# kowallus/mbgc

Hardware: AMD Instinct MI355X
Metric: input Gbases/s (compress hot path, -m1: match-finding + stream emission) (higher is better)
Workload: dtype u8

## Files before the change

mbgc_amd/csrc/swsem_kernels.hip:

```cpp
#include "swsem_device.h"

namespace swk {


__global__ void __launch_bounds__(256) k_load_rc(const uint8_t *__restrict__ src, uint8_t *__restrict__ dst,
                                                 uint64_t n, const uint8_t *__restrict__ lut) {
    __shared__ uint8_t slut[256];
    slut[threadIdx.x] = lut[threadIdx.x];
    __syncthreads();
    const uint64_t stride = (uint64_t) gridDim.x * blockDim.x * 4;
    for (uint64_t d = ((uint64_t) blockIdx.x * blockDim.x + threadIdx.x) * 4; d < n; d += stride) {
        const uint64_t m = n - d < 4 ? n - d : 4;
#pragma unroll
        for (uint64_t k = 0; k < 4; k++)
            if (k < m) dst[d + k] = slut[src[n - 1 - d - k]];
    }
}

__global__ void k_set_byte(uint8_t *p, uint8_t v) { *p = v; }
__global__ void k_touch() {}
__global__ void __launch_bounds__(256) k_hog(unsigned long long ticks) {
    const unsigned long long t0 = __builtin_amdgcn_s_memrealtime();
    while (__builtin_amdgcn_s_memrealtime() - t0 < ticks) __builtin_amdgcn_s_sleep(8);
}
// ... 47 lines not shown
}
__global__ void k_set_bytes(uint8_t *__restrict__ ref, const BytePiece *__restrict__ b, int n, const uint32_t *__restrict__ gate) {
    if (gate && *gate == 0) return;
    for (int i = 0; i < n; i++) ref[b[i].off] = (uint8_t) b[i].val;
}
struct SumRun { uint32_t first, count, val, pad; };
__global__ void __launch_bounds__(256) k_set_tagsum(uint16_t *__restrict__ tagSum, uint32_t nEntries, const SumRun *__restrict__ runs, int n,
                                                    const uint32_t *__restrict__ gate) {
    if (gate && *gate == 0) return;
    for (int i = 0; i < n; i++) {
        const SumRun r = runs[i];
        for (uint32_t k = blockIdx.x * blockDim.x + threadIdx.x; k < r.count; k += gridDim.x * blockDim.x)
            if ((uint64_t) r.first + k < nEntries) tagSum[r.first + k] = (uint16_t) r.val;
    }
}


__device__ __forceinline__ uint32_t fp_at(const uint8_t *s, int nw) {
    uint32_t f = FP_SEED;
    for (int j = 0; j < nw; j++) f = fp_step(f, ld_u32(s + 4 * j));
    return f;
}

__global__ void __launch_bounds__(256) k_insert(const uint8_t *__restrict__ ref, ht_entry *__restrict__ ht,
                                                uint64_t S, uint64_t nMain, uint64_t T, uint64_t nTail, int k1,
                                                int k1ord, int K, uint32_t mask, uint32_t epoch, int fpBits,
                                                uint16_t *__restrict__ tags, uint32_t tag) {
    const uint64_t t = (uint64_t) blockIdx.x * blockDim.x + threadIdx.x;
    if (t >= nMain + nTail) return;
    const bool tail = t >= nMain;
    const uint64_t p = tail ? T + (t - nMain) * (uint64_t) k1 : S + t * (uint64_t) k1;
    if (tags && (p & ((1ull << k1ord) - 1)) == 0) tags[p >> k1ord] = (uint16_t) tag;
    const uint8_t *s = ref + p;
    uint32_t h = (uint32_t) K, f = FP_SEED;
    const int nw = K / 4;
    for (int j = 0; j < nw; j++) { const uint32_t w = ld_u32(s + 4 * j); h = hash_step(h, w, (uint32_t) j); f = fp_step(f, w); }
    const uint32_t off = (uint32_t) (p & ((1ull << k1ord) - 1));
    if (off && p >= off) f = fp_at(s - off, nw);
    const ht_entry key = ht_key(epoch + (tail ? 1u : 0u), (uint32_t) (p >> k1ord), f, fpBits);
    atomicMax(&ht[h & mask], key);
}

struct InsertPiece { uint64_t S, nMain, T, nTail; uint32_t epoch, tag; const uint8_t *src; uint64_t lo, hi; };
__device__ __forceinline__ bool insert_sample(const InsertPiece *__restrict__ pieces, const uint64_t *__restrict__ first, int np, int k1, uint64_t g,
                                              InsertPiece &pc, uint64_t &p, bool &tail) {
    int lo = 0, hi = np;
    while (hi - lo > 1) { const int mid = (lo + hi) / 2; if (first[mid] <= g) lo = mid; else hi = mid; }
    pc = pieces[lo];
    const uint64_t t = g - first[lo];
    tail = t >= pc.nMain;
    p = tail ? pc.T + (t - pc.nMain) * (uint64_t) k1 : pc.S + t * (uint64_t) k1;
    return true;
}
template<bool FROM_SRC>
__global__ void __launch_bounds__(256) k_insert_multi(const uint8_t *__restrict__ ref, ht_entry *__restrict__ ht,
                                                      const InsertPiece *__restrict__ pieces, const uint64_t *__restrict__ first,
                                                      int np, int k1, int k1ord, int K, uint32_t mask, int fpBits,
                                                      const uint32_t *__restrict__ gate, uint16_t *__restrict__ tags) {
    if (gate && *gate == 0) return;
    const uint64_t total = first[np];
    for (uint64_t g0 = (uint64_t) blockIdx.x * blockDim.x + threadIdx.x; g0 < total; g0 += (uint64_t) gridDim.x * blockDim.x) {
        const uint64_t g = total - 1 - g0;
        InsertPiece pc; uint64_t p; bool tail;
        insert_sample(pieces, first, np, k1, g, pc, p, tail);
        const uint8_t *s = ref + p;
        if (FROM_SRC) {
            if (!pc.src || p < pc.lo || p + (uint64_t) K > pc.hi) continue;
            s = pc.src + (p - pc.lo);
        }
        if (tags && (p & ((1ull << k1ord) - 1)) == 0) tags[p >> k1ord] = (uint16_t) pc.tag;
        uint32_t h = (uint32_t) K, f = FP_SEED;
        const int nw = K / 4;
        for (int j = 0; j < nw; j++) { const uint32_t w = ld_u32(s + 4 * j); h = hash_step(h, w, (uint32_t) j); f = fp_step(f, w); }
        const uint32_t off = (uint32_t) (p & ((1ull << k1ord) - 1));
        if (off && p >= off && (!FROM_SRC || p - off >= pc.lo)) f = fp_at(s - off, nw);
        const ht_entry key = ht_key(pc.epoch + (tail ? 1u : 0u), (uint32_t) (p >> k1ord), f, fpBits);
        const ht_entry seen = ht[h & mask];
        if (seen >= key) continue;
        atomicMax(&ht[h & mask], key);
    }
}
__global__ void k_mark_stale(const uint8_t *__restrict__ ref, ht_entry *__restrict__ ht, uint64_t p, int K, int k1ord, uint32_t mask, int fpBits,
                             uint16_t *__restrict__ tags) {
    if (tags) tags[p >> k1ord] = 0;
    uint32_t h = (uint32_t) K;
    for (int j = 0; j < K / 4; j++) h = hash_step(h, ld_u32(ref + p + 4 * j), (uint32_t) j);
    const ht_entry e = ht[h & mask];
    if ((uint32_t) (e >> fpBits) == (uint32_t) (p >> k1ord) && e != 0)
        ht[h & mask] = e & ((((ht_entry) 1) << (32 + fpBits)) - 1);
}

__global__ void __launch_bounds__(256) k_ht_low_words(const ht_entry *__restrict__ ht, uint32_t *__restrict__ out, uint64_t n, int fpBits) {
    const uint64_t i = (uint64_t) blockIdx.x * blockDim.x + threadIdx.x;
    if (i < n) out[i] = (uint32_t) (ht[i] >> fpBits);
}

struct Chain {
    int32_t scan;
    int32_t minTouched;
    int32_t minKeep;
    int32_t visited;
    uint32_t cands;
    bool emitted;
#ifdef SWSEM_DIAG_PHASES
    uint64_t tRefill, tVisit, tLcp;
    uint32_t nRefill, nLcp;
#endif
};
#ifdef SWSEM_DIAG_PHASES
__device__ unsigned long long g_diag[8];
#endif

constexpr int RING = 64;

__device__ __forceinline__ uint32_t rl32(uint32_t x, int lane) { return (uint32_t) __builtin_amdgcn_readlane((int) x, lane); }
__device__ __forceinline__ uint32_t rfl32(uint32_t x) { return (uint32_t) __builtin_amdgcn_readfirstlane((int) x); }
__device__ __forceinline__ uint64_t rfl64(uint64_t x) { return ((uint64_t) rfl32((uint32_t) (x >> 32)) << 32) | rfl32((uint32_t) x); }
constexpr int OVERLAP_MAX = 1024;
constexpr int SNAP = 4;

struct __attribute__((aligned(16))) Row {
    uint64_t posSrc, len, posDest;
    int64_t scanAfter;
};
__device__ __forceinline__ void put_row(Match *dst, const Match &m, int64_t) { *dst = m; }
__device__ __forceinline__ void put_row(Row *dst, const Match &m, int64_t scan) {
    Row r;
    r.posSrc = m.posSrc; r.len = m.len; r.posDest = m.posDest; r.scanAfter = scan;
    *dst = r;
}

template <class R>
// ... 917 lines not shown
```

mbgc_amd/csrc/swsem_runtime_emit.h:

```cpp
namespace {

int end_slot(swsem *h, int si) {
    EmitSlot &E = h->slot[si];
    if (!E.outstanding) return SWSEM_OK;
    HIPCHK(hipSetDevice(h->device));
    { int d = run_phase2b(h, E, false); if (d) return d; }
    HIPCHK(hipEventSynchronize(E.evDone));
    E.outstanding = false;
    const int n = E.emitN;
    E.eout.assign((const EmitOut *) E.pinE.p, (const EmitOut *) E.pinE.p + n);
    uint64_t tot = 0;
    E.hostStreamOff.assign((size_t) n * SWSEM_NSTREAMS, 0);
    for (int k = 0; k < n; k++)
        for (int st = 0; st < SWSEM_NSTREAMS; st++) {
            if (E.eout[k].unmatchedChars == UINT64_MAX) E.eout[k].size[st] = 0;
            E.hostStreamOff[(size_t) k * SWSEM_NSTREAMS + st] = tot;
            tot += E.eout[k].size[st];
        }
    E.packedBytes = tot;
    E.hostStreamsValid = false;
    if (h->emitHostCopy) {
        int r = E.next_host_streams(tot + 1);
        if (r) return r;
        if (tot) HIPCHK(hipMemcpyAsync(E.hostStreams().p, E.dEArena.p, tot, hipMemcpyDeviceToHost, h->s3()));
// ... 62 lines not shown
    h->roundTopFresh = false;
    HIPCHK(hipStreamWaitEvent(up, h->evRoundTop, 0));
    if ((r = upload(h, E.dEOwner.p, E.chunkOwner.data(), E.chunkOwner.size() * sizeof(uint32_t), up))) return r;
    if ((r = upload(h, E.dESpanOwner.p, E.spanOwner.data(), E.spanOwner.size() * sizeof(uint32_t), up))) return r;
    if ((r = upload(h, E.dECg.p, E.ecg.data(), n * sizeof(EmitContig), up)) || (r = upload(h, E.dEWhich.p, E.ewhich.data(), n * sizeof(int), up))) return r;
    E.eloaded.assign(refExtLoadedPos, refExtLoadedPos + nLoaded);
    if ((r = upload(h, E.dELoaded.p, E.eloaded.data(), nLoaded * sizeof(uint64_t), up))) return r;
    if (spec) {
        if ((r = h->dGate.reserve(4)) || (r = h->dPred.reserve(2 * (size_t) n + 64))) return r;
        if ((r = upload(h, h->dPred.p, spec->predExt, n, up)) || (r = upload(h, h->dPred.p + n, spec->predRC, n, up))) return r;
    }
    return flush_copies(h);
}

EmitView emit_book(swsem *h, EmitSlot &E, int si, const swsem_emit_params_t *p, int n, uint64_t nLoaded, bool regionsAhead) {
    EmitView v;
    v.ref = h->ref; v.qbuf = h->qdev; v.matches = h->dMatches.p; v.matchCount = h->dMatchCount.p;
    v.pos1 = (uint64_t) h->ld.pos1; v.refLength = h->refLength(); v.maxRefLength = h->maxRefLength;
    v.loaded = E.dELoaded.p; v.nLoaded = (uint32_t) nLoaded; v.p = *p;
    v.em = E.dEM.p; v.next0 = E.dENext0.p; v.removed = E.dERm.p; v.keepIdx = E.dEKeep.p;
    v.rawLp = regionsAhead ? E.dERawLp.p : nullptr; v.rawNext0 = regionsAhead ? E.dERawNext0.p : nullptr;
    v.meta = E.dEMeta.p; v.corr = E.dECorr.p; v.sz = E.dESz.p; v.arena = E.dEArena.p; v.out = E.dEOut.p;
    v.packBase = E.dEPack.p;
    v.pairMask = E.dEPm.p; v.litBits = E.dELit.p; v.metaBad = E.dEBad.p;
    v.longCopies = E.dELong.p; v.longCount = E.dELongCount.p;
    v.ofs = E.dEOfs.p;
    v.chunkCnt = E.dEChunk.p;
    v.chunkOwner = E.dEOwner.p; v.spanOwner = E.dESpanOwner.p;
    v.ncontigs = (uint32_t) n;
    E.v2b = v; E.grid2b = (uint32_t) E.chunkOwner.size(); E.n2b = n;
    E.donePending = true;
    h->latest = si; h->selected = -1;
    E.outstanding = true; E.refGuarded = false; E.emitN = n; E.emitPos1 = (uint64_t) h->ld.pos1; E.qdev = h->qdev; E.params = *p;
    E.emitLaps = h->ld.laps;
    uint64_t lm = UINT64_MAX; bool all = true;
    for (int k = 0; k < n; k++) { if (E.ecg[k].lock == UINT64_MAX) all = false; else lm = std::min(lm, E.ecg[k].lock); }
    E.lockMin = all ? lm : UINT64_MAX;
    E.packedBytes = 0; E.hostStreamsValid = false;
    E.deferred2b = false;
    return v;
}

int spec_plan(swsem *h, const swsem_spec_finalize_t *spec, const uint32_t *gate, bool &planned) {
    h->specMode = true;
    int r = finalize_impl(h, spec->ntargets, spec->ext_dev, spec->ext_len, spec->addSep, spec->sep, spec->lazySeparator, spec->lockPos,
                          spec->loadedAfter, gate, true);
    h->specMode = false;
    planned = r == SWSEM_OK;
    if (r == SWSEM_ESPEC) return SWSEM_OK;
    if (r) return r;
    return prepare_inserts(h, h->streamUp);
}

int emit_pass1(swsem *h, EmitSlot &E, const EmitView &v, int n) {
    const dim3 grid2(E.grid2b);
    int r;
    HIPCHK(hipEventRecord(h->evTables, h->streamUp));
    if (v.rawLp) {
        HIPCHK(hipStreamWaitEvent(h->streamAux, h->evMatched, 0));
        HIPCHK(hipStreamWaitEvent(h->streamAux, h->evTables, 0));
        k_emit_regions_raw<<<grid2, dim3(CH), 0, h->streamAux>>>(v, E.dECg.p, E.dEWhich.p);
        HIPCHK(hipEventRecord(h->evRegions, h->streamAux));
    }
    HIPCHK(hipStreamWaitEvent(h->stream, h->evTables, 0));
    hipStream_t sP = h->stream;
    h->mark(SWSEM_K_EMIT, true, sP);
    k_emit_p1_removed<<<grid2, dim3(CH), 0, sP>>>(v, E.dECg.p, E.dEWhich.p);
    k_emit_p1_scan<<<dim3(n), dim3(CH), 0, sP>>>(v, E.dECg.p, E.dEWhich.p);
    if (v.rawLp) HIPCHK(hipStreamWaitEvent(sP, h->evRegions, 0));
    k_emit_p1_compact<<<grid2, dim3(CH), 0, sP>>>(v, E.dECg.p, E.dEWhich.p);
    k_emit_p1_finish<<<dim3(n), dim3(CH), 0, sP>>>(v, E.dECg.p);
    h->mark(SWSEM_K_EMIT, false, sP);
    HIPCHK(hipGetLastError());
    if ((r = queue_counts(h, n * sizeof(EmitOut), sP))) return r;
    if ((r = download(h, h->pin.p + h->pinExtraAt, E.dEOut.p, n * sizeof(EmitOut), sP)) || (r = flush_copies(h))) return r;
    HIPCHK(hipEventRecord(h->evP1, sP));
    return SWSEM_OK;
}

int emit_pairing(swsem *h, EmitSlot &E, const EmitView &v, int n) {
    const dim3 grid2(E.grid2b), spans((uint32_t) E.spanOwner.size());
    const size_t outBytes = n * sizeof(EmitOut);
    int r = E.pinE.reserve(outBytes, std::max<size_t>(2 * outBytes, 1 << 20));
    if (r) return r;
    HIPCHK(hipStreamWaitEvent(h->streamAux, h->evP1, 0));
    h->mark(SWSEM_K_EMIT2, true, h->streamAux);
    if (!v.rawLp) k_emit_meta_regions<<<grid2, dim3(CH), 0, h->streamAux>>>(v, E.dECg.p);
    k_emit_meta_masks<<<spans, dim3(MLANES), 0, h->streamAux>>>(v, E.dECg.p);
    k_emit_meta_spec<<<spans, dim3(MLANES), 0, h->streamAux>>>(v, E.dECg.p, E.dEStates.p, h->sw.metaWarm, E.dEStat.p);
    HIPCHK(hipEventRecord(h->evMeta, h->streamAux));
    h->metaPending = true;
    k_emit_meta_check<<<grid2, dim3(WAVE), 0, h->streamAux>>>(v, E.dECg.p, E.dEStates.p, E.dEStat.p);
    k_emit_meta_stitch<<<dim3(n), dim3(WAVE), 0, h->streamAux>>>(v, E.dECg.p, E.dEStates.p, E.dEStat.p);
    h->mark(SWSEM_K_EMIT2, false, h->streamAux);
    HIPCHK(hipEventRecord(E.evMetaDone, h->streamAux));
    HIPCHK(hipGetLastError());
    return SWSEM_OK;
}

int spec_gate(swsem *h, EmitSlot &E, const swsem_spec_finalize_t *spec, uint32_t *gate, int n, bool planned, bool &queued, bool &exchanged) {
    k_spec_verify<<<1, 256, 0, h->stream>>>(E.dEOut.p, E.dECg.p, n, h->dPred.p, h->dPred.p + n, spec->factor, spec->rcFactor, gate);
    if (spec->veto || !planned) HIPCHK(hipMemsetAsync(gate, 0, sizeof(uint32_t), h->stream));
    if (spec->exchange) {
        if (spec->exchange(spec->exchange_ctx, 0, gate, (void *) h->stream)) return fail(SWSEM_EHIP, "speculative finalize: the exchange between the replicas failed");
        exchanged = true;
    }
    if (planned) {
        int r = launch_inserts(h, gate);
        if (r) return r;
        queued = true;
    }
    return SWSEM_OK;
}

bool spec_verdict(swsem *h, const EmitSlot &E, const swsem_spec_finalize_t *spec, int n, bool exchanged) {
    bool ok = !spec->veto;
    for (int k = 0; k < n && ok; k++) {
        const uint64_t un = E.eout[k].unmatchedChars, len = E.ecg[k].n;
        ok = un != UINT64_MAX && (un * (uint64_t) spec->factor > len) == (spec->predExt[k] != 0) &&
             (un * (uint64_t) spec->rcFactor > len) == (spec->predRC[k] != 0);
    }
    if (exchanged) ok = spec->exchange(spec->exchange_ctx, 1, nullptr, (void *) h->stream) == 1 && ok;
    return ok;
}

int emit_begin_impl(swsem *h, const swsem_emit_params_t *p, int n, const int *contigIdx, const uint64_t *lockPos,
                    const int *factor, const int64_t *processed, const int64_t *targetIdx,
                    const uint64_t *refExtLoadedPos, uint64_t nLoaded, const swsem_spec_finalize_t *spec, int *applied) {
    HIPCHK(hipSetDevice(h->device));
    if (applied) *applied = 0;
    if (spec && spec->ntargets <= 0) spec = nullptr;
    const int si = h->latest ^ 1;
    { int e = end_slot(h, si); if (e) return e; }
    EmitSlot &E = h->slot[si];
    if (!h->batchValid) return fail(SWSEM_EINVAL, "swsem_emit: no match results on the handle");
    if (n <= 0) return fail(SWSEM_EINVAL, "swsem_emit: empty request");
    if (p->lazyDecompressionSupport && nLoaded == 0) return fail(SWSEM_EINVAL, "swsem_emit: lazy mode needs refExtLoadedPosArr");
    if (p->gapDepthOffsetEncoding > 64 || p->gapDepthOffsetEncoding < 0)
        return fail(SWSEM_EINVAL, "gapDepthOffsetEncoding %d out of range (MAX_GAP_DEPTH / 2)", p->gapDepthOffsetEncoding);
    int r;
    uint64_t rows, arena;
    const bool regionsAhead = h->roundTopFresh && p->lazyDecompressionSupport;
    if ((r = emit_layout(h, E, n, contigIdx, lockPos, factor, processed, targetIdx, rows, arena)) ||
        (r = emit_reserve(h, E, n, rows, arena, nLoaded)) ||
        (r = emit_upload_tables(h, E, n, refExtLoadedPos, nLoaded, spec)))
        return r;
    const EmitView v = emit_book(h, E, si, p, n, nLoaded, regionsAhead);
    const LoaderState snap = h->ld;
    bool planned = false, queued = false, exchanged = false;
    uint32_t *gate = spec ? (spec->gate_dev ? spec->gate_dev : h->dGate.p) : nullptr;
    if (spec && (r = spec_plan(h, spec, gate, planned))) return r;
    const bool needCounts = h->matchCount.size() != h->contigs.size();
    if ((r = emit_pass1(h, E, v, n))) return r;
    if ((r = emit_pairing(h, E, v, n))) return r;
    if (spec) {
        if ((r = spec_gate(h, E, spec, gate, n, planned, queued, exchanged))) return r;
        if (!queued) h->ld = snap;
    }
    E.deferred2b = true; E.waitFin2b = queued;
    if (h->emitHostCopy) { int e = end_slot(h, si ^ 1); if (e) return e; }
    HIPCHK(hipEventSynchronize(h->evP1));
    if (needCounts) take_counts(h);
    E.eout.assign((const EmitOut *) (h->pin.p + h->pinExtraAt), (const EmitOut *) (h->pin.p + h->pinExtraAt) + n);
    if (queued) {
        if (spec_verdict(h, E, spec, n, exchanged)) { if (applied) *applied = 1; }
        else h->ld = snap;
    } else if (exchanged)
        (void) spec->exchange(spec->exchange_ctx, 1, nullptr, (void *) h->stream);
    return SWSEM_OK;
}

}
```

mbgc_amd/csrc/swsem_runtime_loader.h:

```cpp
namespace {

int flush_copies(swsem *h) {
    CopySegs &sg = h->segs;
    if (sg.n == 0) return SWSEM_OK;
    const uint32_t blocks = sg.first[sg.n];
    k_copy_segs<<<dim3(blocks), dim3(256), 0, h->segStream>>>(sg);
    sg.n = 0;
    HIPCHK(hipGetLastError());
    return SWSEM_OK;
}
int stage_copy(swsem *h, void *dst, const void *src, size_t bytes, hipStream_t st) {
    if (!bytes) return SWSEM_OK;
    CopySegs &sg = h->segs;
    if (sg.n && (h->segStream != st || sg.n == CopySegs::MAX)) { int r = flush_copies(h); if (r) return r; }
    if (sg.n == 0) { h->segStream = st; sg.first[0] = 0; }
    sg.dst[sg.n] = (uint8_t *) dst; sg.src[sg.n] = (const uint8_t *) src; sg.bytes[sg.n] = bytes;
    sg.first[sg.n + 1] = sg.first[sg.n] + (uint32_t) ((bytes + 4095) / 4096);
    sg.n++;
    return SWSEM_OK;
}
int download(swsem *h, void *dstPinned, const void *srcDev, size_t bytes, hipStream_t st) { return stage_copy(h, dstPinned, srcDev, bytes, st); }
int zero_dev(swsem *h, void *dst, size_t bytes, hipStream_t st) { return stage_copy(h, dst, nullptr, bytes, st); }

int upload(swsem *h, void *dst, const void *src, size_t bytes, hipStream_t st) {
// ... 232 lines not shown
    P = PreparedInserts();
    const size_t np = h->pendingPieces.size(), nc = h->pendingCopies.size(), nb = h->pendingBytes.size();
    plan_tag_summary(h, h->sumRuns);
    const size_t ns = h->sumRuns.size();
    P.np = np; P.nc = nc; P.nb = nb; P.ns = ns;
    if (!np && !nc && !nb && !ns) return SWSEM_OK;
    constexpr uint64_t CHUNK = 256 * 16;
    std::vector<InsertPiece> &edge = h->edgePieces;
    edge.clear();
    bool beside = np && nc;
    for (size_t i = 0; i < nc && beside; i++)
        for (size_t j = i + 1; j < nc && beside; j++)
            beside = h->pendingCopies[i].dst + h->pendingCopies[i].len <= h->pendingCopies[j].dst || h->pendingCopies[j].dst + h->pendingCopies[j].len <= h->pendingCopies[i].dst;
    if (beside) {
        const int64_t k1 = h->k1, K = h->K;
        for (auto &pc : h->pendingPieces) {
            if (pc.src)
                for (auto &b : h->pendingBytes)
                    if (b.off >= pc.lo && b.off < pc.hi) { if (b.off - pc.lo < pc.hi - b.off) { pc.src += b.off + 1 - pc.lo; pc.lo = b.off + 1; } else pc.hi = b.off; }
            auto runs = [&](uint64_t base, uint64_t n, uint32_t epoch) {
                if (!n) return;
                int64_t a = 0, b = -1;
                if (pc.src && (int64_t) pc.hi - K >= (int64_t) base) {
                    a = (int64_t) pc.lo > (int64_t) base ? ((int64_t) pc.lo - (int64_t) base + k1 - 1) / k1 : 0;
                    b = std::min<int64_t>((int64_t) n - 1, ((int64_t) pc.hi - K - (int64_t) base) / k1);
                }
                auto push = [&](int64_t t0, int64_t t1) {
                    if (t1 <= t0) return;
                    InsertPiece e = {};
                    e.S = base + (uint64_t) t0 * (uint64_t) k1; e.nMain = (uint64_t) (t1 - t0); e.epoch = epoch; e.tag = pc.tag;
                    edge.push_back(e);
                };
                if (b < a) push(0, (int64_t) n);
                else { push(0, a); push(b + 1, (int64_t) n); }
            };
            runs(pc.S, pc.nMain, pc.epoch);
            runs(pc.T, pc.nTail, pc.epoch + 1);
        }
    } else
        for (auto &pc : h->pendingPieces) pc.src = nullptr;
    const size_t ne = edge.size();
    const size_t wPieces = np * (sizeof(InsertPiece) / 8), wCopies = nc * (sizeof(CopyPiece) / 8), wBytes = nb * (sizeof(BytePiece) / 8), wEdge = ne * (sizeof(InsertPiece) / 8),
                 wSums = ns * (sizeof(SumRun) / 8);
    swsem::HostTab &ht = h->hostTables[h->hostTableSel ^= 1];
    const size_t words = wPieces + (np + 1) + wCopies + (nc + 1) + wBytes + wEdge + (ne + 1) + wSums;
    if (ht.pending) { HIPCHK(hipEventSynchronize(ht.ev)); ht.pending = false; }
    int r;
    if ((r = ht.buf.reserve(words * 8, std::max<size_t>(2 * words, 1 << 16) * 8))) return r;
    uint64_t *const tab = (uint64_t *) ht.buf.p;
    uint64_t *tPieces = tab, *tFirst = tPieces + wPieces, *tCopies = tFirst + np + 1, *tCFirst = tCopies + wCopies, *tBytes = tCFirst + nc + 1,
             *tEdge = tBytes + wBytes, *tEFirst = tEdge + wEdge, *tSums = tEFirst + ne + 1;
    if (np) memcpy(tPieces, h->pendingPieces.data(), np * sizeof(InsertPiece));
    tFirst[0] = 0;
    for (size_t i = 0; i < np; i++) tFirst[i + 1] = tFirst[i] + h->pendingPieces[i].nMain + h->pendingPieces[i].nTail;
    if (nc) memcpy(tCopies, h->pendingCopies.data(), nc * sizeof(CopyPiece));
    tCFirst[0] = 0;
    for (size_t i = 0; i < nc; i++) tCFirst[i + 1] = tCFirst[i] + (h->pendingCopies[i].len + CHUNK - 1) / CHUNK;
    if (nb) memcpy(tBytes, h->pendingBytes.data(), nb * sizeof(BytePiece));
    if (ne) memcpy(tEdge, edge.data(), ne * sizeof(InsertPiece));
    tEFirst[0] = 0;
    for (size_t i = 0; i < ne; i++) tEFirst[i + 1] = tEFirst[i] + edge[i].nMain;
    if (ns) memcpy(tSums, h->sumRuns.data(), ns * sizeof(SumRun));
    if ((r = h->dTables.reserve(std::max<size_t>(2 * words, 1 << 16)))) return r;
    k_upload<<<dim3((unsigned) ((words * 8 + 4095) / 4096)), dim3(256), 0, upStream>>>((uint8_t *) h->dTables.p, (const uint8_t *) tab, words * 8);
    HIPCHK(hipEventRecord(ht.ev, upStream));
    ht.pending = true;
    const uint64_t *d = h->dTables.p;
    P.beside = beside; P.ne = ne;
    P.nSamples = tFirst[np]; P.nEdge = tEFirst[ne]; P.copyBlocks = tCFirst[nc];
    P.dPieces = (const InsertPiece *) (d + (tPieces - tab)); P.dFirst = d + (tFirst - tab);
    P.dCopies = (const CopyPiece *) (d + (tCopies - tab)); P.dCFirst = d + (tCFirst - tab);
    P.dBytes = (const BytePiece *) (d + (tBytes - tab));
    P.dEdge = (const InsertPiece *) (d + (tEdge - tab)); P.dEFirst = d + (tEFirst - tab);
    P.dSums = (const SumRun *) (d + (tSums - tab));
    h->pendingPieces.clear(); h->pendingCopies.clear(); h->pendingBytes.clear();
    HIPCHK(hipGetLastError());
    return SWSEM_OK;
}

int launch_inserts(swsem *h, const uint32_t *gate) {
    hipStream_t sV = h->stream;
    PreparedInserts &P = h->prep;
    const size_t np = P.np, nc = P.nc, nb = P.nb, ne = P.ne, ns = P.ns;
    if (!np && !nc && !nb && !ns) return SWSEM_OK;
    hipStream_t cs = sV;
    if (P.beside) {
        cs = h->streamLoad;
        HIPCHK(hipEventRecord(h->evLoadFork, sV));
        HIPCHK(hipStreamWaitEvent(cs, h->evLoadFork, 0));
    }
    if (nc) {
        h->mark(SWSEM_K_LOAD, true, cs);
        k_copy_multi<<<dim3((unsigned) std::min<uint64_t>(P.copyBlocks, COPY_WGS)), dim3(256), 0, cs>>>(h->ref, P.dCopies, P.dCFirst, (int) nc, gate);
        h->mark(SWSEM_K_LOAD, false, cs);
    }
    if (nb) k_set_bytes<<<1, 1, 0, cs>>>(h->ref, P.dBytes, (int) nb, gate);
    if (ns) k_set_tagsum<<<dim3(16), dim3(256), 0, cs>>>(h->tagSum, h->tagSumEntries, P.dSums, (int) ns, gate);
    if (P.beside) HIPCHK(hipEventRecord(h->evLoadDone, cs));
    if (np && P.nSamples) {
        h->mark(SWSEM_K_INSERT, true);
        const dim3 grid((unsigned) ((P.nSamples + 255) / 256));
        if (P.beside) k_insert_multi<true><<<grid, dim3(256), 0, h->stream>>>(h->ref, h->ht, P.dPieces, P.dFirst, (int) np, h->k1, h->k1ord, h->K, h->mask, h->fpBits, gate, h->tags);
        else k_insert_multi<false><<<grid, dim3(256), 0, h->stream>>>(h->ref, h->ht, P.dPieces, P.dFirst, (int) np, h->k1, h->k1ord, h->K, h->mask, h->fpBits, gate, h->tags);
        h->mark(SWSEM_K_INSERT, false);
    }
    if (P.beside) {
        HIPCHK(hipStreamWaitEvent(h->stream, h->evLoadDone, 0));
        if (ne && P.nEdge)
            k_insert_multi<false><<<dim3((unsigned) ((P.nEdge + 255) / 256)), dim3(256), 0, h->stream>>>(
                h->ref, h->ht, P.dEdge, P.dEFirst, (int) ne, h->k1, h->k1ord, h->K, h->mask, h->fpBits, gate, h->tags);
    }
    HIPCHK(hipGetLastError());
    return SWSEM_OK;
}

int flush_inserts(swsem *h, const uint32_t *gate) {
    int r = prepare_inserts(h, h->stream);
    return r ? r : launch_inserts(h, gate);
}
int flush_tag_summary(swsem *h) {
    if (h->sumUniform.empty() && h->sumMixed.empty()) return SWSEM_OK;
    return flush_inserts(h);
}

int load_separator(swsem *h, int sep) {
    LoaderState &ld = h->ld;
    ld.wrap_if_at_end(h->maxRefLength);
    if ((uint64_t) ld.pos1 == h->maxRefLength) return SWSEM_OK;
    if ((uint64_t) ld.pos1 == ld.swEnd && ld.sep_end_done(sep)) return SWSEM_OK;
    { const uint64_t at = (uint64_t) ld.pos1 == ld.swEnd ? (uint64_t) ld.pos1 - 1 : (uint64_t) ld.pos1; int g = ref_write_guard(h, at, at); if (g) return g; }
    if ((uint64_t) ld.pos1 == ld.swEnd) {
        if (h->specMode) return SWSEM_ESPEC;
        if (h->deferInserts) { int r = flush_inserts(h); if (r) return r; }
        if (ld.pos1 >= (int64_t) h->K + REF_SHIFT)
            k_mark_stale<<<1, 1, 0, h->stream>>>(h->ref, h->ht, (uint64_t) (ld.pos1 - h->K), h->K, h->k1ord, h->mask, h->fpBits, h->tags);
        k_set_byte<<<1, 1, 0, h->stream>>>(h->ref + ld.pos1 - 1, (uint8_t) sep);
        note_byte(h, (uint64_t) ld.pos1 - 1);
        ld.sep_end_set(ld.pos1, sep);
    } else if (h->deferInserts) {
        { int f = flush_if_hit(h, (uint64_t) ld.pos1, (uint64_t) ld.pos1 + 1); if (f) return f; }
        note_byte(h, (uint64_t) ld.pos1);
        BytePiece bp; bp.off = (uint64_t) ld.pos1++; bp.val = (uint64_t) (uint8_t) sep;
        h->pendingBytes.push_back(bp);
    } else {
        note_byte(h, (uint64_t) ld.pos1);
        k_set_byte<<<1, 1, 0, h->stream>>>(h->ref + ld.pos1++, (uint8_t) sep);
    }
    HIPCHK(hipGetLastError());
    return h->deferInserts ? SWSEM_OK : flush_tag_summary(h);
}

uint64_t loaded_ref_length(const swsem *h) {
    return (uint64_t) h->ld.laps * (h->maxRefLength - REF_SHIFT) + ((uint64_t) h->ld.pos1 - REF_SHIFT);
}

int release_lock(swsem *h, uint64_t v) {
    if (h->swSize == 0 || !h->circular) return SWSEM_OK;
    std::deque<uint64_t> &locks = h->ld.locks;
    size_t i = 0;
    while (i < locks.size() && locks[i] != v) i++;
// ... 31 lines not shown
```

mbgc_amd/csrc/swsem_runtime_state.h:

```cpp
#define SWSEM_ESPEC (-100)

namespace {

thread_local std::string g_err;
int fail(int code, const char *fmt, ...) {
    char buf[512];
    va_list ap;
    va_start(ap, fmt);
    vsnprintf(buf, sizeof buf, fmt, ap);
    va_end(ap);
    g_err = buf;
    return code;
}
#define HIPCHK(x) do { hipError_t e_ = (x); if (e_ != hipSuccess) return fail(SWSEM_EHIP, "%s: %s", #x, hipGetErrorString(e_)); } while (0)

constexpr uint64_t REF_SHIFT = 1;
constexpr int SW_WIDTH_FACTOR = 16;
constexpr uint64_t REF_SLACK = 256;
constexpr uint64_t COPY_WGS = 2048;
constexpr uint32_t EMIT_THIN_MAX = 512;
constexpr uint32_t RB_MIN = 2048 / RBU;
constexpr uint32_t CAND_MAX = 4096;
constexpr uint64_t CAND_BYTES = 128ull << 20;
constexpr int NSTATS = 16;

struct NoCopy {
    NoCopy() = default;
    NoCopy(const NoCopy &) = delete;
    NoCopy &operator=(const NoCopy &) = delete;
};
template <typename T>
struct DevBuf : NoCopy {
    T *p = nullptr;
    size_t cap = 0;
    ~DevBuf() { if (p) (void) hipFree(p); }
    int reserve(size_t n) {
        if (n <= cap) return SWSEM_OK;
        if (p) (void) hipFree(p);
        p = nullptr; cap = 0;
        size_t want = n + n / 8 + 64;
        if (hipMalloc((void **) &p, want * sizeof(T)) != hipSuccess) {
            p = nullptr;
            return fail(SWSEM_ENOMEM, "device allocation of %zu bytes failed", want * sizeof(T));
        }
        cap = want;
        return SWSEM_OK;
    }
};

struct PinBuf : NoCopy {
    uint8_t *p = nullptr;
    size_t cap = 0;
    ~PinBuf() { if (p) (void) hipHostFree(p); }
    int reserve(size_t bytes, size_t want, unsigned flags = hipHostMallocCoherent | hipHostMallocMapped) {
        if (bytes <= cap) return SWSEM_OK;
        if (p) (void) hipHostFree(p);
        p = nullptr; cap = 0;
        if (hipHostMalloc((void **) &p, want, flags) != hipSuccess) {
            p = nullptr;
            return fail(SWSEM_ENOMEM, "cannot pin %zu B of host memory", want);
        }
        cap = want;
        return SWSEM_OK;
    }
};

thread_local bool g_eventsFailed = false;
struct Event : NoCopy {
    hipEvent_t e = nullptr;
    Event() { if (hipEventCreateWithFlags(&e, hipEventDisableTiming) != hipSuccess) { e = nullptr; g_eventsFailed = true; } }
    ~Event() { if (e) (void) hipEventDestroy(e); }
    operator hipEvent_t() const { return e; }
// ... 7 lines not shown
    uint64_t samplingPos = 0, swEnd = 0;
    std::deque<uint64_t> locks;
    uint32_t epoch = 1;
    uint32_t eCur = 0, ePrev = 0;
    int64_t sepEndPos = -1; int sepEndLaps = -1, sepEndVal = -1;
    bool pristine = true;
    uint64_t droppedBytes = 0;

    bool sep_end_done(int sep) const { return pos1 == sepEndPos && laps == sepEndLaps && sep == sepEndVal; }
    void sep_end_set(int64_t at, int sep) { sepEndPos = at; sepEndLaps = laps; sepEndVal = sep; }
    uint64_t refLength(uint64_t maxRefLength) const { return laps ? maxRefLength : (uint64_t) pos1; }
    void wrap_if_at_end(uint64_t maxRefLength) {
        if ((uint64_t) pos1 != maxRefLength || swEnd == maxRefLength) return;
        laps++;
        ePrev = eCur; eCur = epoch;
        pos1 = REF_SHIFT;
        samplingPos = REF_SHIFT;
    }
};

struct Switches {
    bool seqResolve = false;
    bool simt = true;
    uint32_t rbFixed = 0;
    int overlapFixed = -1;
    uint32_t profMask = ~0u;
    int metaWarm = swk::MWARM;
    bool lapTags = true;
    int tagSumShift = 12;
    bool streamCalib = true;
    bool streamDebug = false;
    bool debugStats = false;
};
Switches read_switches() {
    Switches s;
    if (const char *e = getenv("SWSEM_RESOLVE")) s.seqResolve = strcmp(e, "seq") == 0;
    if (const char *e = getenv("SWSEM_CHAINS")) s.simt = atoi(e) != 1;
    if (const char *e = getenv("SWSEM_RB")) { int x = atoi(e); if (x >= 1 && x <= 256) s.rbFixed = (uint32_t) x * (1024 / RBU); }
    if (const char *e = getenv("SWSEM_OVERLAP")) { int x = atoi(e); if (x >= 0 && x <= swk::OVERLAP_MAX) s.overlapFixed = x; }
    if (const char *e = getenv("SWSEM_PROF_FAMS")) s.profMask = (uint32_t) strtoul(e, nullptr, 0);
    if (const char *e = getenv("SWSEM_META_WARM")) s.metaWarm = std::min(swk::MWARM, std::max(0, atoi(e)));
    if (const char *e = getenv("SWSEM_LAP_TAGS")) s.lapTags = atoi(e) != 0;
    if (const char *e = getenv("SWSEM_TAGSUM_SHIFT")) { int x = atoi(e); if (x >= 0 && x <= 24) s.tagSumShift = x; }
    if (const char *e = getenv("SWSEM_STREAM_CALIB")) s.streamCalib = atoi(e) != 0;
    s.streamDebug = getenv("SWSEM_STREAM_DEBUG") != nullptr;
    s.debugStats = getenv("SWSEM_DEBUG_STATS") != nullptr;
    return s;
}

struct PreparedInserts {
    size_t np = 0, nc = 0, nb = 0, ne = 0, ns = 0;
    const SumRun *dSums = nullptr;
    bool beside = false;
    uint64_t nSamples = 0, nEdge = 0, copyBlocks = 0;
    const InsertPiece *dPieces = nullptr, *dEdge = nullptr;
    const uint64_t *dFirst = nullptr, *dCFirst = nullptr, *dEFirst = nullptr;
    const CopyPiece *dCopies = nullptr;
    const BytePiece *dBytes = nullptr;
};

struct EmitSlot {
    DevBuf<EmitContig> dECg;
    DevBuf<EmitOut> dEOut;
    DevBuf<int> dEWhich;
    DevBuf<uint32_t> dEOwner, dESpanOwner;
    DevBuf<EMatch> dEM;
    DevBuf<uint64_t> dENext0, dELoaded, dEPack;
    DevBuf<uint64_t> dERawLp, dERawNext0;
    DevBuf<uint8_t> dERm, dEArena;
    DevBuf<uint32_t> dEKeep, dEMeta, dECorr, dESz, dEOfs, dEChunk;
    DevBuf<MetaRec> dEStates;
    DevBuf<unsigned long long> dEStat, dEPm, dELit, dEBad;
    DevBuf<LongCopy> dELong;
    DevBuf<uint32_t> dELongCount;
    bool statZeroed = false;
    std::vector<EmitContig> ecg;
    std::vector<uint32_t> chunkOwner, spanOwner;
    std::vector<int> ewhich;
    std::vector<uint64_t> eloaded;
    std::vector<EmitOut> eout;
    Event evDone;
    Event evMetaDone;
    bool outstanding = false, refGuarded = false;
    bool donePending = false;
    bool deferred2b = false, waitFin2b = false;
    EmitView v2b; uint32_t grid2b = 0; int n2b = 0;
    const uint8_t *qdev = nullptr;
    swsem_emit_params_t params;
    uint64_t emitPos1 = 0;
    uint64_t lockMin = UINT64_MAX;
    int emitLaps = 0;
    int emitN = 0;
    PinBuf pinE;
    PinBuf hostHalf[2];
    int hostAt = 0;
    PinBuf &hostStreams() { return hostHalf[hostAt]; }
    int next_host_streams(size_t n) { hostAt ^= 1; return hostStreams().reserve(n, n + n / 2 + 4096, hipHostMallocDefault); }
    std::vector<uint64_t> hostStreamOff;
    bool hostStreamsValid = false;
    uint64_t packedBytes = 0;
};

}

struct swsem {
    int device = 0;
    hipStream_t stream = nullptr;
    bool ownStream = false;
    Switches sw;
    uint8_t *ref = nullptr;
    ht_entry *ht = nullptr;
    uint8_t *lut = nullptr;
    uint16_t *tags = nullptr;
    bool useTags = true;
    uint16_t *tagSum = nullptr;
    int tagSumShift = 0;
    uint32_t tagSumEntries = 0;
    struct SumSpan { uint64_t a, b; uint32_t val; };
    std::vector<SumSpan> sumUniform, sumMixed;
    std::vector<SumRun> sumRuns;
    LoaderState ld;
    uint64_t maxRefLength = 0;
    int L = 0, K = 0, k1 = 0, skipMargin = 0, k1ord = 0;
    uint32_t hash_size = 0, mask = 0;
    uint64_t swSize = 0;
    bool circular = true;
    int fpBits = 0;
    uint64_t hostProbes = 0;
    bool deferInserts = false;
    bool specMode = false;
    DevBuf<uint32_t> dGate;
    DevBuf<uint8_t> dPred;
    std::vector<InsertPiece> pendingPieces;
    std::vector<InsertPiece> edgePieces;
    int prioLow = 0, prioHigh = 0;
    Event evLoadFork, evLoadDone;
    std::vector<CopyPiece> pendingCopies;
    std::vector<BytePiece> pendingBytes;
    DevBuf<uint64_t> dTables;
    struct HostTab { PinBuf buf; Event ev; bool pending = false; } hostTables[2];
    int hostTableSel = 0;
    PreparedInserts prep;
    hipStream_t stream2 = nullptr, streamLoad = nullptr, streamUp = nullptr, streamAux = nullptr;
    Event evTables, evRoundTop;
    bool roundTopFresh = false;
    DevBuf<uint8_t> stage;
    DevBuf<Contig> dContigs;
    DevBuf<uint32_t> dMatchCount, dRbContig, dRbOrder;
    std::vector<uint32_t> rbOrderHost, rbOrderKey;
    uint32_t chainsPerWave = 1;
    hipStream_t stream3 = nullptr;
    hipStream_t s3() {
        if (!stream3 && hipStreamCreateWithFlags(&stream3, hipStreamNonBlocking) != hipSuccess) stream3 = stream;
        return stream3;
    }
    Event evMatched;
    std::vector<uint32_t> rbContigHost;
    DevBuf<Match> dMatches;
    DevBuf<Row> dRegions, dReplay;
    DevBuf<BlockRec> dRecs;
    DevBuf<FastRec> dFast;
    DevBuf<uint32_t> dCandOf, dCandBlock;
    DevBuf<CandRec> dCand;
    DevBuf<Row> dCandArea;
    DevBuf<uint32_t> dSegStart, dKeepN, dDstOff;
    DevBuf<int32_t> dPrev;
    DevBuf<unsigned long long> dStats;
    DevBuf<uint8_t> dDecode;
    DevBuf<DecodeJob> dJobs;
    DevBuf<DecRec> dDecRecs;
    DevBuf<DecPlanOut> dDecPlan;
    DevBuf<uint64_t> dDecAux;
    bool decoder = false;
    struct ChainState {
        DevBuf<ChainStart> dStarts;
        DevBuf<ChainContig> dContigs;
        DevBuf<uint32_t> dSeqCount, dChainBad, dBad;
        DevBuf<uint64_t> dLock, dRecBase;
        DevBuf<LoadSeg> dSegs;
        DevBuf<ProvRow> dProv;
        DevBuf<uint64_t> dTime;
        DevBuf<uint32_t> dNeed;
        DevBuf<ProvRowG> dProvG;
        DevBuf<uint32_t> dNeedG;
        DevBuf<uint64_t> dGranBase;
        uint32_t granShift = 0;
        uint64_t regionFor = 0;
        ChainStreams streams = {};
        swsem_emit_params_t params = {};
        uint64_t n = 0;
        std::vector<uint64_t> nrec, destLen, litEnd, lock;
        const uint8_t *jobsDest = nullptr;
    } chain;
    EmitSlot slot[2];
    int latest = 0;
// ... 80 lines not shown
```

Measured before the change: 58.68.

## Insert hash-table samples speculatively before gate, with undo log on veto

The hash-table insert kernel now launches right after the tables are ready, before the speculative gate is decided. Emit pass 1 and verification move to the load stream so they can run alongside it. Each insert logs the old bucket value and tag, and a new undo kernel restores them if the gate ends up zero. The aim is to take the insert off the critical path after verification, at the cost of a per-sample log write, an undo pass, and more complex cross-stream ordering where the loader copies and the early inserts may now race.

```diff
diff --git a/mbgc_amd/csrc/swsem_kernels.hip b/mbgc_amd/csrc/swsem_kernels.hip
--- a/mbgc_amd/csrc/swsem_kernels.hip
+++ b/mbgc_amd/csrc/swsem_kernels.hip
@@ -123,11 +123,13 @@
     p = tail ? pc.T + (t - pc.nMain) * (uint64_t) k1 : pc.S + t * (uint64_t) k1;
     return true;
 }
-template<bool FROM_SRC>
+struct __attribute__((aligned(16))) InsertLog { ht_entry old; uint32_t bucket; uint16_t tag, flags; };
+template<bool FROM_SRC, bool LOG = false>
 __global__ void __launch_bounds__(256) k_insert_multi(const uint8_t *__restrict__ ref, ht_entry *__restrict__ ht,
                                                       const InsertPiece *__restrict__ pieces, const uint64_t *__restrict__ first,
                                                       int np, int k1, int k1ord, int K, uint32_t mask, int fpBits,
-                                                      const uint32_t *__restrict__ gate, uint16_t *__restrict__ tags) {
+                                                      const uint32_t *__restrict__ gate, uint16_t *__restrict__ tags,
+                                                      InsertLog *__restrict__ log = nullptr) {
     if (gate && *gate == 0) return;
     const uint64_t total = first[np];
     for (uint64_t g0 = (uint64_t) blockIdx.x * blockDim.x + threadIdx.x; g0 < total; g0 += (uint64_t) gridDim.x * blockDim.x) {
@@ -136,9 +138,14 @@
         insert_sample(pieces, first, np, k1, g, pc, p, tail);
         const uint8_t *s = ref + p;
         if (FROM_SRC) {
-            if (!pc.src || p < pc.lo || p + (uint64_t) K > pc.hi) continue;
+            if (!pc.src || p < pc.lo || p + (uint64_t) K > pc.hi) {
+                if (LOG) log[g0] = InsertLog{0, 0u, 0, 0};
+                continue;
+            }
             s = pc.src + (p - pc.lo);
         }
+        InsertLog rec = {0, 0u, 0, 0};
+        if (LOG && tags && (p & ((1ull << k1ord) - 1)) == 0) { rec.tag = tags[p >> k1ord]; rec.flags = 2; }
         if (tags && (p & ((1ull << k1ord) - 1)) == 0) tags[p >> k1ord] = (uint16_t) pc.tag;
         uint32_t h = (uint32_t) K, f = FP_SEED;
         const int nw = K / 4;
@@ -147,8 +154,27 @@
         if (off && p >= off && (!FROM_SRC || p - off >= pc.lo)) f = fp_at(s - off, nw);
         const ht_entry key = ht_key(pc.epoch + (tail ? 1u : 0u), (uint32_t) (p >> k1ord), f, fpBits);
         const ht_entry seen = ht[h & mask];
+        if (LOG) {
+            if (seen < key) { rec.old = seen; rec.bucket = h & mask; rec.flags |= 1; }
+            log[g0] = rec;
+        }
         if (seen >= key) continue;
         atomicMax(&ht[h & mask], key);
+    }
+}
+__global__ void __launch_bounds__(256) k_insert_undo(ht_entry *__restrict__ ht, const InsertPiece *__restrict__ pieces, const uint64_t *__restrict__ first,
+                                                     int np, int k1, int k1ord, int fpBits, const uint32_t *__restrict__ gate,
+                                                     uint16_t *__restrict__ tags, const InsertLog *__restrict__ log, uint32_t epoch0) {
+    if (*gate != 0) return;
+    const uint64_t total = first[np];
+    for (uint64_t g0 = (uint64_t) blockIdx.x * blockDim.x + threadIdx.x; g0 < total; g0 += (uint64_t) gridDim.x * blockDim.x) {
+        const InsertLog e = log[g0];
+        if ((e.flags & 1) && (uint32_t) (e.old >> (32 + fpBits)) < epoch0) ht[e.bucket] = e.old;
+        if (e.flags & 2) {
+            InsertPiece pc; uint64_t p; bool tail;
+            insert_sample(pieces, first, np, k1, total - 1 - g0, pc, p, tail);
+            tags[p >> k1ord] = e.tag;
+        }
     }
 }
 __global__ void k_mark_stale(const uint8_t *__restrict__ ref, ht_entry *__restrict__ ht, uint64_t p, int K, int k1ord, uint32_t mask, int fpBits,
diff --git a/mbgc_amd/csrc/swsem_runtime_emit.h b/mbgc_amd/csrc/swsem_runtime_emit.h
--- a/mbgc_amd/csrc/swsem_runtime_emit.h
+++ b/mbgc_amd/csrc/swsem_runtime_emit.h
@@ -138,7 +138,7 @@
     return prepare_inserts(h, h->streamUp);
 }
 
-int emit_pass1(swsem *h, EmitSlot &E, const EmitView &v, int n) {
+int emit_pass1(swsem *h, EmitSlot &E, const EmitView &v, int n, bool insertEarly, hipStream_t &sP) {
     const dim3 grid2(E.grid2b);
     int r;
     HIPCHK(hipEventRecord(h->evTables, h->streamUp));
@@ -149,7 +149,15 @@
         HIPCHK(hipEventRecord(h->evRegions, h->streamAux));
     }
     HIPCHK(hipStreamWaitEvent(h->stream, h->evTables, 0));
-    hipStream_t sP = h->stream;
+    sP = h->stream;
+    if (insertEarly) {
+        HIPCHK(hipEventRecord(h->evLoadFork, h->stream));
+        if ((r = launch_insert_early(h))) return r;
+        if (h->prep.early) {
+            sP = h->streamLoad;
+            HIPCHK(hipStreamWaitEvent(sP, h->evLoadFork, 0));
+        }
+    }
     h->mark(SWSEM_K_EMIT, true, sP);
     k_emit_p1_removed<<<grid2, dim3(CH), 0, sP>>>(v, E.dECg.p, E.dEWhich.p);
     k_emit_p1_scan<<<dim3(n), dim3(CH), 0, sP>>>(v, E.dECg.p, E.dEWhich.p);
@@ -184,15 +192,15 @@
     return SWSEM_OK;
 }
 
-int spec_gate(swsem *h, EmitSlot &E, const swsem_spec_finalize_t *spec, uint32_t *gate, int n, bool planned, bool &queued, bool &exchanged) {
-    k_spec_verify<<<1, 256, 0, h->stream>>>(E.dEOut.p, E.dECg.p, n, h->dPred.p, h->dPred.p + n, spec->factor, spec->rcFactor, gate);
-    if (spec->veto || !planned) HIPCHK(hipMemsetAsync(gate, 0, sizeof(uint32_t), h->stream));
+int spec_gate(swsem *h, EmitSlot &E, const swsem_spec_finalize_t *spec, uint32_t *gate, int n, bool planned, hipStream_t sV, bool &queued, bool &exchanged) {
+    k_spec_verify<<<1, 256, 0, sV>>>(E.dEOut.p, E.dECg.p, n, h->dPred.p, h->dPred.p + n, spec->factor, spec->rcFactor, gate);
+    if (spec->veto || !planned) HIPCHK(hipMemsetAsync(gate, 0, sizeof(uint32_t), sV));
     if (spec->exchange) {
-        if (spec->exchange(spec->exchange_ctx, 0, gate, (void *) h->stream)) return fail(SWSEM_EHIP, "speculative finalize: the exchange between the replicas failed");
+        if (spec->exchange(spec->exchange_ctx, 0, gate, (void *) sV)) return fail(SWSEM_EHIP, "speculative finalize: the exchange between the replicas failed");
         exchanged = true;
     }
     if (planned) {
-        int r = launch_inserts(h, gate);
+        int r = launch_inserts(h, gate, sV);
         if (r) return r;
         queued = true;
     }
@@ -237,10 +245,11 @@
     uint32_t *gate = spec ? (spec->gate_dev ? spec->gate_dev : h->dGate.p) : nullptr;
     if (spec && (r = spec_plan(h, spec, gate, planned))) return r;
     const bool needCounts = h->matchCount.size() != h->contigs.size();
-    if ((r = emit_pass1(h, E, v, n))) return r;
+    hipStream_t sP = h->stream;
+    if ((r = emit_pass1(h, E, v, n, spec && planned && !spec->exchange, sP))) return r;
     if ((r = emit_pairing(h, E, v, n))) return r;
     if (spec) {
-        if ((r = spec_gate(h, E, spec, gate, n, planned, queued, exchanged))) return r;
+        if ((r = spec_gate(h, E, spec, gate, n, planned, sP, queued, exchanged))) return r;
         if (!queued) h->ld = snap;
     }
     E.deferred2b = true; E.waitFin2b = queued;
diff --git a/mbgc_amd/csrc/swsem_runtime_loader.h b/mbgc_amd/csrc/swsem_runtime_loader.h
--- a/mbgc_amd/csrc/swsem_runtime_loader.h
+++ b/mbgc_amd/csrc/swsem_runtime_loader.h
@@ -308,7 +308,11 @@
              *tEdge = tBytes + wBytes, *tEFirst = tEdge + wEdge, *tSums = tEFirst + ne + 1;
     if (np) memcpy(tPieces, h->pendingPieces.data(), np * sizeof(InsertPiece));
     tFirst[0] = 0;
-    for (size_t i = 0; i < np; i++) tFirst[i + 1] = tFirst[i] + h->pendingPieces[i].nMain + h->pendingPieces[i].nTail;
+    uint32_t epoch0 = UINT32_MAX;
+    for (size_t i = 0; i < np; i++) {
+        tFirst[i + 1] = tFirst[i] + h->pendingPieces[i].nMain + h->pendingPieces[i].nTail;
+        epoch0 = std::min(epoch0, h->pendingPieces[i].epoch);
+    }
     if (nc) memcpy(tCopies, h->pendingCopies.data(), nc * sizeof(CopyPiece));
     tCFirst[0] = 0;
     for (size_t i = 0; i < nc; i++) tCFirst[i + 1] = tCFirst[i] + (h->pendingCopies[i].len + CHUNK - 1) / CHUNK;
@@ -323,7 +327,7 @@
     ht.pending = true;
     const uint64_t *d = h->dTables.p;
     P.beside = beside; P.ne = ne;
-    P.nSamples = tFirst[np]; P.nEdge = tEFirst[ne]; P.copyBlocks = tCFirst[nc];
+    P.nSamples = tFirst[np]; P.nEdge = tEFirst[ne]; P.copyBlocks = tCFirst[nc]; P.epoch0 = epoch0;
     P.dPieces = (const InsertPiece *) (d + (tPieces - tab)); P.dFirst = d + (tFirst - tab);
     P.dCopies = (const CopyPiece *) (d + (tCopies - tab)); P.dCFirst = d + (tCFirst - tab);
     P.dBytes = (const BytePiece *) (d + (tBytes - tab));
@@ -334,16 +338,32 @@
     return SWSEM_OK;
 }
 
-int launch_inserts(swsem *h, const uint32_t *gate) {
-    hipStream_t sV = h->stream;
+int launch_insert_early(swsem *h) {
+    PreparedInserts &P = h->prep;
+    if (!P.beside || !P.np || !P.nSamples) return SWSEM_OK;
+    int r = h->dInsLog.reserve(P.nSamples);
+    if (r) return r;
+    h->mark(SWSEM_K_INSERT, true);
+    k_insert_multi<true, true><<<dim3((unsigned) std::min<uint64_t>((P.nSamples + 255) / 256, INSERT_WGS)), dim3(256), 0, h->stream>>>(
+        h->ref, h->ht, P.dPieces, P.dFirst, (int) P.np, h->k1, h->k1ord, h->K, h->mask, h->fpBits, nullptr, h->tags, h->dInsLog.p);
+    h->mark(SWSEM_K_INSERT, false);
+    HIPCHK(hipGetLastError());
+    P.early = true;
+    return SWSEM_OK;
+}
+
+int launch_inserts(swsem *h, const uint32_t *gate, hipStream_t sV = nullptr) {
+    if (!sV) sV = h->stream;
     PreparedInserts &P = h->prep;
     const size_t np = P.np, nc = P.nc, nb = P.nb, ne = P.ne, ns = P.ns;
     if (!np && !nc && !nb && !ns) return SWSEM_OK;
     hipStream_t cs = sV;
     if (P.beside) {
         cs = h->streamLoad;
-        HIPCHK(hipEventRecord(h->evLoadFork, sV));
-        HIPCHK(hipStreamWaitEvent(cs, h->evLoadFork, 0));
+        if (sV != cs) {
+            HIPCHK(hipEventRecord(h->evLoadFork, sV));
+            HIPCHK(hipStreamWaitEvent(cs, h->evLoadFork, 0));
+        }
     }
     if (nc) {
         h->mark(SWSEM_K_LOAD, true, cs);
@@ -353,7 +373,11 @@
     if (nb) k_set_bytes<<<1, 1, 0, cs>>>(h->ref, P.dBytes, (int) nb, gate);
     if (ns) k_set_tagsum<<<dim3(16), dim3(256), 0, cs>>>(h->tagSum, h->tagSumEntries, P.dSums, (int) ns, gate);
     if (P.beside) HIPCHK(hipEventRecord(h->evLoadDone, cs));
-    if (np && P.nSamples) {
+    if (P.early) {
+        HIPCHK(hipStreamWaitEvent(h->stream, h->evLoadDone, 0));
+        k_insert_undo<<<dim3((unsigned) std::min<uint64_t>((P.nSamples + 255) / 256, UNDO_WGS)), dim3(256), 0, h->stream>>>(
+            h->ht, P.dPieces, P.dFirst, (int) np, h->k1, h->k1ord, h->fpBits, gate, h->tags, h->dInsLog.p, P.epoch0);
+    } else if (np && P.nSamples) {
         h->mark(SWSEM_K_INSERT, true);
         const dim3 grid((unsigned) ((P.nSamples + 255) / 256));
         if (P.beside) k_insert_multi<true><<<grid, dim3(256), 0, h->stream>>>(h->ref, h->ht, P.dPieces, P.dFirst, (int) np, h->k1, h->k1ord, h->K, h->mask, h->fpBits, gate, h->tags);
@@ -361,7 +385,7 @@
         h->mark(SWSEM_K_INSERT, false);
     }
     if (P.beside) {
-        HIPCHK(hipStreamWaitEvent(h->stream, h->evLoadDone, 0));
+        if (!P.early) HIPCHK(hipStreamWaitEvent(h->stream, h->evLoadDone, 0));
         if (ne && P.nEdge)
             k_insert_multi<false><<<dim3((unsigned) ((P.nEdge + 255) / 256)), dim3(256), 0, h->stream>>>(
                 h->ref, h->ht, P.dEdge, P.dEFirst, (int) ne, h->k1, h->k1ord, h->K, h->mask, h->fpBits, gate, h->tags);
diff --git a/mbgc_amd/csrc/swsem_runtime_state.h b/mbgc_amd/csrc/swsem_runtime_state.h
--- a/mbgc_amd/csrc/swsem_runtime_state.h
+++ b/mbgc_amd/csrc/swsem_runtime_state.h
@@ -18,6 +18,8 @@
 constexpr int SW_WIDTH_FACTOR = 16;
 constexpr uint64_t REF_SLACK = 256;
 constexpr uint64_t COPY_WGS = 2048;
+constexpr uint64_t INSERT_WGS = 2048;
+constexpr uint64_t UNDO_WGS = 1024;
 constexpr uint32_t EMIT_THIN_MAX = 512;
 constexpr uint32_t RB_MIN = 2048 / RBU;
 constexpr uint32_t CAND_MAX = 4096;
@@ -131,6 +133,8 @@
     size_t np = 0, nc = 0, nb = 0, ne = 0, ns = 0;
     const SumRun *dSums = nullptr;
     bool beside = false;
+    bool early = false;
+    uint32_t epoch0 = 0;
     uint64_t nSamples = 0, nEdge = 0, copyBlocks = 0;
     const InsertPiece *dPieces = nullptr, *dEdge = nullptr;
     const uint64_t *dFirst = nullptr, *dCFirst = nullptr, *dEFirst = nullptr;
@@ -220,6 +224,7 @@
     struct HostTab { PinBuf buf; Event ev; bool pending = false; } hostTables[2];
     int hostTableSel = 0;
     PreparedInserts prep;
+    DevBuf<InsertLog> dInsLog;
     hipStream_t stream2 = nullptr, streamLoad = nullptr, streamUp = nullptr, streamAux = nullptr;
     Event evTables, evRoundTop;
     bool roundTopFresh = false;
diff --git a/profiles/insert_gap.py b/profiles/insert_gap.py
--- /dev/null
+++ b/profiles/insert_gap.py
@@ -0,0 +1,47 @@
+#!/usr/bin/env python3
+import csv, glob, json, statistics, sys
+
+f = glob.glob(sys.argv[1] + "/**/*kernel_trace.csv", recursive=True)[0]
+K = int(sys.argv[2])
+rows = sorted(csv.DictReader(open(f)), key=lambda r: int(r["Start_Timestamp"]))
+for r in rows:
+    r["s"], r["e"], r["n"] = int(r["Start_Timestamp"]), int(r["End_Timestamp"]), r["Kernel_Name"]
+idx = [i for i, r in enumerate(rows) if "k_resolve_blocks4" in r["n"]]
+idx = idx[-(K + 1):]
+P1 = ("k_emit_p1_removed", "k_emit_p1_scan", "k_emit_p1_compact", "k_emit_p1_finish", "k_emit_regions_raw", "k_spec_verify")
+OTHER = ("k_insert_multi<true", "k_insert_multi<false", "k_insert_undo", "k_copy_multi", "k_stitch_pre", "k_stitch_replay", "k_stitch<", "k_gather")
+steps = []
+for a, b in zip(idx[:-1], idx[1:]):
+    seg = rows[a:b]
+    t0, nxt = rows[a]["s"], rows[b]["s"]
+    def sel(name):
+        return [r for r in seg if name in r["n"]]
+    gat, ins = sel("k_gather"), sel("k_insert_multi<true")
+    p1a, p1b = sel("k_emit_p1_removed"), sel("k_spec_verify")
+    st = {"wrapped": "<true>" in rows[a]["n"].split("k_resolve_blocks4")[1][:8], "step_us": (nxt - t0) / 1e3}
+    if gat and ins:
+        ge, i0, i1 = max(r["e"] for r in gat), min(r["s"] for r in ins), max(r["e"] for r in ins)
+        st["gather_end_to_insert_start_us"] = (i0 - ge) / 1e3
+        st["insert_end_to_next_resolve_us"] = (nxt - i1) / 1e3
+        st["gather_end_to_next_resolve_us"] = (nxt - ge) / 1e3
+        if p1a and p1b:
+            pa, pb = min(r["s"] for r in p1a), max(r["e"] for r in p1b)
+            st["pass1_us"] = (pb - pa) / 1e3
+            st["insert_beside_pass1_us"] = max(0, min(i1, pb) - max(i0, pa)) / 1e3
+    for name in P1 + OTHER:
+        v = [(r["e"] - r["s"]) / 1e3 for r in sel(name)]
+        st["dur_" + name] = round(sum(v), 1) if v else None
+    steps.append(st)
+
+def summ(vals):
+    vals = [v for v in vals if v is not None]
+    if not vals:
+        return None
+    return {"n": len(vals), "min": round(min(vals), 1), "median": round(statistics.median(vals), 1), "max": round(max(vals), 1)}
+
+keys = sorted({k for s in steps for k in s if k != "wrapped"})
+out = {}
+for tag, part in (("before_wrap", [s for s in steps if not s["wrapped"]]), ("after_wrap", [s for s in steps if s["wrapped"]]), ("all", steps)):
+    out[tag] = {k: summ([s.get(k) for s in part]) for k in keys} if part else None
+out["steps"] = steps
+json.dump(out, sys.stdout, indent=1)
```

New measurement: 56.77. 0.967x the previous value.
